# tayloraswift/swift-png

Hardware: AMD Instinct MI355X
Metric: decoded_mpixels_per_s (higher is better)
Workload: dtype u8

## Files before the change

### swift_png_amd/csrc/pinflate2.hip

```cpp
#include "common.hpp"
#include <type_traits>
#include <cstddef>
#include "huffman.hpp"

namespace spng {

#ifdef SPNG_EMU
#define AS_GLOBAL
#else
#define AS_GLOBAL __attribute__((address_space(1)))
#endif
__device__ __forceinline__ uint32_t mul24(uint32_t a, uint32_t b)
{
#ifdef SPNG_EMU
    return (a & 0xffffffu) * (b & 0xffffffu);
#else
    uint32_t r;
    asm("v_mul_u32_u24 %0, %1, %2" : "=v"(r) : "v"(a), "v"(b));
    return r;
#endif
}
typedef uint32_t v4u __attribute__((vector_size(16)));
struct __attribute__((packed)) PV4 { v4u v; };
typedef uint8_t AS_GLOBAL g8;
// ... 1061 lines not shown
__global__ __launch_bounds__(64) void pinf2_cutplan_kernel(PStream *__restrict__ streams, PSeg *__restrict__ segs, PCut *__restrict__ cuts, uint32_t *__restrict__ stats)
{
    __shared__ __attribute__((aligned(16))) DLds s;
    const int lane = threadIdx.x;
    PStream &st = streams[blockIdx.x];
    const uint32_t need = UNI(st.cut_segs);
    if (!need || UNI(st.serial_only)) return;
    const uint32_t first = UNI(st.seg_first), count = UNI(st.seg_count);
    const g8 *src = (const g8 *)uni64((uint64_t)st.src);
    const uint64_t n = uni64(st.src_len), sb = uni64(st.seg_bytes), org = uni64(st.seg_origin);
    const bool rcut = UNI(st.cut_resumed) != 0;
    {
        uint32_t prev = ~0u;
        for (uint32_t base = 0; base < count; base += 64) {
            const uint32_t i = base + (uint32_t)lane;
            unsigned long long mask = __ballot(i < count && segs[first + i].start_bit != NONE2);
            while (mask) {
                const uint32_t f = base + (uint32_t)__ffsll((long long)mask) - 1;
                mask &= mask - 1;
                bool keep = true;
                if (prev != ~0u && f - prev - 1 >= need) {
                    const uint64_t at = uni64(segs[first + f].start_bit);
                    Hdr2 h;
                    if (UB(parse_header2(s, src, n, uni64(segs[first + prev].start_bit), h, lane)) && h.type != 0) {
                        uint32_t len = 0, code = 0;
                        for (uint32_t k = 0; k < (1u << LB) / 64; ++k) {
                            const uint32_t idx = k * 64 + (uint32_t)lane, e = s.lit[idx];
                            const unsigned long long m = __ballot(((e >> 5) & 7) == C_EOB);
                            if (m && !len) {
                                const int l = __ffsll((long long)m) - 1;
                                len = (uint32_t)__shfl((int)((e >> 8) & 15), l, 64);
                                code = (k * 64 + (uint32_t)l) & ((1u << len) - 1);
                            }
                        }
                        if (len && at >= len) {
                            const uint64_t b = at - len;
                            uint32_t v = 0;
                            for (uint32_t k = 0; k < 3; ++k) if ((b >> 3) + k < n) v |= (uint32_t)src[(b >> 3) + k] << (8 * k);
                            keep = ((v >> (b & 7)) & ((1u << len) - 1)) == code;
                        }
                    }
                }
                if (keep) prev = f;
                else if (lane == 0) segs[first + f].start_bit = NONE2;
            }
        }
        __threadfence();
    }
    uint32_t carry = ~0u;
    for (uint32_t base = 0; base < count; base += 64) {
        const uint32_t i = base + (uint32_t)lane;
        const bool has = i < count && segs[first + i].start_bit != NONE2;
        const unsigned long long mask = __ballot(has);
        const unsigned long long low = mask & ((2ull << lane) - 1);
        if (i < count) cuts[first + i].anchor = low ? base + 63 - (uint32_t)__clzll((long long)low) : carry;
        if (mask) carry = base + 63 - (uint32_t)__clzll((long long)mask);
    }
    uint32_t nxt = count, tried = 0;
    for (uint32_t base = (count - 1) & ~63u;; base -= 64) {
        const uint32_t i = base + (uint32_t)lane;
        const bool has = i < count && segs[first + i].start_bit != NONE2;
        const unsigned long long mask = __ballot(has);
        const unsigned long long high = mask >> lane;
        const uint32_t nf = high ? i + (uint32_t)__ffsll((long long)high) - 1 : nxt;
        bool cut = false;
        if (i < count && !has) {
            const uint32_t a = cuts[first + i].anchor;
            if (a != ~0u) {
                const uint64_t lo = org + (uint64_t)(a + 1) * sb, hi = org + (uint64_t)nf * sb < n ? org + (uint64_t)nf * sb : n;
                const uint64_t b = segs[first + a].start_bit;
                const uint64_t from = a == 0 && rcut ? org : lo;
                if (hi > lo && hi - from >= (uint64_t)need * sb && b + 3 <= n * 8) {
                    const uint32_t v = (uint32_t)src[b >> 3] | ((b >> 3) + 1 < n ? (uint32_t)src[(b >> 3) + 1] << 8 : 0u);
                    const uint32_t type = (v >> ((b & 7) + 1)) & 3;
                    cut = type == 1 || type == 2;
                }
            }
            cuts[first + i].cut = cut ? 1u : 0u;
        }
        tried += (uint32_t)__popcll(__ballot(cut));
        if (mask) nxt = base + (uint32_t)__ffsll((long long)mask) - 1;
        if (base == 0) break;
    }
    if (lane == 0 && tried) { atomicAdd(stats, tried); st.cut_on = 1; }
    if (!tried && uni64(st.tok_bit)) back_to_the_header(st, segs, lane);
}

__global__ __launch_bounds__(64, SPNG_D_WAVES) void pinf2_cutjoin_kernel(const PStream *__restrict__ streams, PSeg *__restrict__ segs,
                                                                        PCut *__restrict__ cuts, uint32_t *__restrict__ pt_slab, DPool pool, uint32_t seg0,
                                                                        uint32_t *__restrict__ stats)
{
    __shared__ __attribute__((aligned(16))) DLds s;
    const int lane = threadIdx.x;
    const PSeg &pd = segs[seg0 + blockIdx.x];
    PCut &pc = cuts[seg0 + blockIdx.x];
    if ((int32_t)UNI(pd.status) != PSEG_CUT) return;
    const PStream &st = streams[UNI(pd.stream)];
    const uint32_t j = UNI(pd.next);
    if (j <= UNI(pd.index) || j >= UNI(st.seg_count)) return;
    const PCut &sg = cuts[UNI(st.seg_first) + j];
    const uint32_t nrec = UNI(sg.nrec);
    if (!UNI(sg.cut) || !nrec) return;
    const g8 *src = (const g8 *)uni64((uint64_t)st.src);
    const uint64_t n = uni64(st.src_len);
    const uint64_t want = uni64(sg.head_tbl);
    uint64_t pos = uni64(pd.end_bit), id = uni64(pc.tbl_id);
    g32 *pt = (g32 *)(pt_slab + uni64(pd.log_off));
    const uint32_t pt_cap = uni64(pd.log_cap) > 0xffffff00ull ? 0xffffff00u : (uint32_t)uni64(pd.log_cap);
    Cursor cur;
    cur.nhw = uni64(pd.ntok); cur.npages = (uint32_t)((cur.nhw + PAGE_HW - 1) >> (PAGE_SHIFT - 1)); cur.dry = false;
    cur.pa = (cur.nhw & (PAGE_HW - 1)) ? (g8 *)(pool.base + ((uint64_t)UNI(pt[cur.nhw >> (PAGE_SHIFT - 1)]) << PAGE_SHIFT)) : nullptr;
    const uint64_t hw0 = cur.nhw;
    uint64_t nbytes = 0;
    uint32_t c = 0, chunks = 0;
    bool mid = true, have = false, ok = false;
    uint64_t jt = 0, jt_bytes = 0;
    Hdr2 h;
    for (uint32_t steps = 0; steps < 4 * CUT_JOIN_CHUNKS; ++steps) {
        while (c < nrec && uni64(sg.rec[c].bit) < pos) ++c;
        if (c == nrec) break;
        if (mid && uni64(sg.rec[c].bit) == pos) { ok = id == want; break; }
        if (chunks == CUT_JOIN_CHUNKS) break;
        if (!have || !mid) {
            const uint64_t at = mid ? uni64(pc.tbl) : pos;
            if (!UB(parse_header2(s, src, n, at, h, lane)) || h.type == 0) break;
            have = true;
            if (!mid) { id = table_id(h, pos); jt = pos; jt_bytes = nbytes; pos = h.payload; mid = true; continue; }
        }
        const uint32_t sdw = chunk_dwords(h.minlen);
        const uint64_t chb = (uint64_t)sdw * 32 * 64, upto = uni64(sg.rec[c].bit);
        uint64_t next;
        const uint32_t state = cut_chunk<true>(s, h, src, n, pos, pos, sdw, pool, pt, pt_cap, cur, next, nbytes, upto - pos < chb ? upto : pos + chb, lane);
        chunks += 1;
        if (state == 2) break;
        pos = uni64(next);
        if (state == 1) { if (h.bfinal) break; mid = false; }
    }
    if (!ok) return;
    if (chunks > 1) COV(7);
    if (lane == 0) {
        pc.add_tok = cur.nhw - hw0; pc.add_bytes = nbytes;
        pc.next_head = UNI(sg.rec[c].hw); pc.next_sub = UNI(sg.rec[c].bytes); pc.joined = 1;
        pc.next_bit = pos; pc.join_tbl = jt; pc.join_tbl_bytes = jt_bytes;
        atomicAdd(stats + 1, 1u);
    }
}

template <uint32_t RETRY, bool CUT>
__device__ __forceinline__ void scan_stream(PStream *__restrict__ streams, PSeg *__restrict__ segs, PPart *__restrict__ parts, uint32_t *__restrict__ stats,
                                            const PCut *__restrict__ cuts)
{
    constexpr uint32_t retry = RETRY;
    const int lane = threadIdx.x;
    PStream &st = streams[blockIdx.x];
    if (retry && UNI(st.pass) != 1) {
        if (lane == 0) st.ok = 0;
        return;
    }
    const uint32_t first = UNI(st.seg_first), count = UNI(st.seg_count);
    bool ok = false, partial = false, dry = false;
    uint64_t tok = 0, end_bit = 0, out = 0;
    uint32_t k = 0;
    bool met_cut = false, by_cut = false;
    uint32_t skip_hw = 0; uint64_t skip_bytes = 0;
    const bool rcut = CUT && UNI(st.cut_resumed) != 0;
    uint64_t cur_hdr = CUT ? uni64(st.start_bit) : 0, cur_out = CUT ? uni64(st.blk_out) : 0, ho_bit = 0;
    bool handed = false;
    for (uint32_t hops = 0; hops < count; ++hops) {
        PSeg *sg = segs + first + k;
        const uint64_t start = uni64(sg->start_bit), end = uni64(sg->end_bit);
        const int32_t status = (int32_t)UNI(sg->status);
        if (status == PSEG_NOPAGE && (start != NONE2 || (CUT && by_cut))) dry = true;
        if ((start == NONE2 && !(CUT && by_cut)) || status == PSEG_FAIL || status == PSEG_NOPAGE) break;
        if constexpr (CUT) {
            uint64_t nt = uni64(sg->ntok), nb = uni64(sg->nbytes);
            const uint32_t hd = by_cut ? skip_hw : 0u;
            if (by_cut) nb -= skip_bytes;
            uint32_t nx = 0;
            if (status == PSEG_CUT) {
                met_cut = true;
                nx = UNI(sg->next);
                const PCut &ct = cuts[first + k];
                const bool joined = nx > k && nx < count && UNI(cuts[first + nx].cut) && UNI(ct.joined);
                if (rcut) {
                    if (UNI(ct.tbl_here)) { cur_hdr = uni64(ct.tbl); cur_out = uni64(st.out_pos) + out + uni64(ct.tbl_bytes) - (by_cut ? skip_bytes : 0); }
                    if (!joined || (int32_t)UNI(segs[first + nx].status) == PSEG_FAIL) {
                        ho_bit = end;
                        if (joined) {
                            if (uni64(ct.join_tbl)) { cur_hdr = uni64(ct.join_tbl); cur_out = uni64(st.out_pos) + out + nb + uni64(ct.join_tbl_bytes); }
                            nt += uni64(ct.add_tok); nb += uni64(ct.add_bytes); ho_bit = uni64(ct.next_bit);
                        }
                        if (lane == 0) { sg->tok_base = tok; sg->out_base = out; sg->used = 1; sg->ntok = nt; sg->nbytes = nb; sg->head = hd; sg->status = PSEG_PARTIAL; }
                        tok += nt - hd; out += nb;
                        handed = true;
                        break;
                    }
                    if (uni64(ct.join_tbl)) { cur_hdr = uni64(ct.join_tbl); cur_out = uni64(st.out_pos) + out + nb + uni64(ct.join_tbl_bytes); }
                }
                if (!joined) break;
                nt += uni64(ct.add_tok); nb += uni64(ct.add_bytes);
                skip_hw = UNI(ct.next_head); skip_bytes = uni64(ct.next_sub);
            }
            if (lane == 0) { sg->tok_base = tok; sg->out_base = out; sg->used = 1; sg->ntok = nt; sg->nbytes = nb; sg->head = hd; }
            tok += nt - hd;
            out += nb;
            if (status == PSEG_CUT) { k = nx; by_cut = true; continue; }
            by_cut = false;
        } else {
        if (lane == 0) { sg->tok_base = tok; sg->out_base = out; sg->used = 1; }
        tok += uni64(sg->ntok);
        out += uni64(sg->nbytes);
        }
        if (status == PSEG_FINAL) { ok = true; end_bit = end; break; }
        if (status == PSEG_PARTIAL) { ok = true; partial = true; end_bit = end; break; }
        const uint32_t nx = UNI(sg->next);
        if (nx <= k || nx >= count) break;
        if (uni64(segs[first + nx].start_bit) != end) break;
        k = nx;
    }
    if (CUT && handed && uni64(st.src_len) * 8 - ho_bit <= 2 * uni64(st.seg_bytes) * 8) { ok = true; partial = true; end_bit = ho_bit; }
    else handed = false;
    if (CUT && met_cut && !(ok && (!partial || rcut))) {
        ok = false; partial = false; dry = true; handed = false;
        if (lane == 0) atomicAdd(stats + 2, 1u);
        COV(8);
    }
    bool again = !retry && dry;
    if constexpr (CUT) { if (again && uni64(st.tok_bit)) again = back_to_the_header(st, segs, lane); }
    const uint32_t pmax = UNI(st.parts_max);
    uint32_t np = 0;
    if (pmax > 1 && ok && uni64(st.start_bit) == 0 && uni64(st.out_pos) == 0 && out <= uni64(st.dst_cap) && out > 0) {
        PPart *pp = parts + (uint64_t)blockIdx.x * pmax;
        uint64_t w0 = (uint64_t)gridDim.x * (pmax - 1) > 256 ? 1 : 0;
#ifdef SPNG_EMU
        if (getenv("EMU_FIRST_PART_SHARE")) w0 = 1;
#endif
        uint64_t begun = 0;
        uint32_t kk = 0, tnext = 1;
        np = 1;
        if (lane == 0) { pp[0].seg = 0; pp[0].out_pos = 0; pp[0].present = 1; }
        for (uint32_t hops = 0; hops < count; ++hops) {
            const PSeg *sg = segs + first + kk;
            const uint64_t ob = uni64(sg->out_base);
            if (kk != 0 && tnext < pmax && ob >= 32768u && ob > begun && ob * (2 * pmax + w0) >= (uint64_t)(2 * tnext + w0) * out) {
                if (lane == 0) {
                    pp[np].seg = kk; pp[np].out_pos = ob; pp[np].present = 1;
                    pp[np - 1].seg_end = kk; pp[np - 1].out_len = ob - begun;
                }
                begun = ob; np += 1;
                tnext = (uint32_t)((ob * (2 * pmax + w0) / out + 2 - w0) / 2);
            }
            if ((int32_t)UNI(sg->status) == PSEG_FINAL || (int32_t)UNI(sg->status) == PSEG_PARTIAL) break;
            kk = UNI(sg->next);
        }
        if (lane == 0) { pp[np - 1].seg_end = ~0u; pp[np - 1].out_len = out - begun; }
    }
    if (lane == 0) { st.ok = ok ? (handed ? 3 : partial ? 2 : 1) : 0; st.ntok = tok; st.end_bit = end_bit; st.pass = again ? 1 : 0; st.tok_base = 0;
                     st.out_total = out; st.parts = np; st.ho_hdr = cur_hdr; st.ho_out = cur_out; }
}

template <uint32_t RETRY>
__global__ __launch_bounds__(64) void pinf2_scan_kernel(PStream *__restrict__ streams, PSeg *__restrict__ segs, PPart *__restrict__ parts)
{
    scan_stream<RETRY, false>(streams, segs, parts, nullptr, nullptr);
}
__global__ __launch_bounds__(64) void pinf2_cutscan_kernel(PStream *__restrict__ streams, PSeg *__restrict__ segs, const PCut *__restrict__ cuts,
                                                           PPart *__restrict__ parts, uint32_t *__restrict__ stats)
{
    scan_stream<0, true>(streams, segs, parts, stats, cuts);
}

#ifndef SPNG_R_THREADS
#define SPNG_R_THREADS 512
#define SPNG_R_WAVES 4
#endif
static constexpr uint32_t RT2 = SPNG_R_THREADS;
static constexpr uint32_t NW2 = RT2 / 64;
template <bool BIG> struct RGeo {
    static constexpr uint32_t TILE = BIG ? 8192 : 4096;
    static constexpr uint32_t BPT = TILE / RT2;
    static constexpr uint32_t HPT = TILE / 2 / RT2;
    static constexpr uint32_t EB = BPT < 8 ? BPT : 8;
    static constexpr uint32_t MAXM = TILE / 8;
};
static constexpr uint32_t WINDOW2 = 32768;
static constexpr uint32_t R2_DONE = 0x8000;
static constexpr uint32_t PTC = 256;

template <bool MARK> struct RingOf { typedef uint8_t T; };
template <> struct RingOf<true> { typedef uint16_t T; };
template <bool MARK, bool BIG>
struct RLds2T {
    typename RingOf<MARK>::T ring[WINDOW2];
    uint16_t state[RGeo<BIG>::TILE];
    uint32_t rec[RGeo<BIG>::MAXM + 2][2];
    uint32_t bitmap[RGeo<BIG>::TILE / 32];
    uint16_t h0[RT2 + 8];
    uint32_t pt[PTC];
    uint32_t part[3 * NW2];
    uint32_t cut[2];
};

template <class L>
__device__ __forceinline__ uint32_t block_excl_scan2(L &s, uint32_t v, uint32_t &total, int tid)
{
    const int lane = tid & 63, wave = tid >> 6;
    uint32_t wt;
    const uint32_t off = wave_excl_scan(v, wt, lane);
    if (lane == 0) s.part[wave] = wt;
    __syncthreads();
    uint32_t before = 0, all = 0;
#pragma unroll
    for (int w4 = 0; w4 < (int)NW2; w4 += 4) {
        const v4u p = *(const v4u *)(s.part + w4);
#pragma unroll
        for (int c = 0; c < 4; ++c) { before += w4 + c < wave ? p[c] : 0u; all += p[c]; }
    }
    total = all;
    return off + before;
}

__device__ __forceinline__ void stream_verdict(const PStream &st, uint32_t S, uint32_t I, uint64_t pos, spng_result *__restrict__ results,
                                               int32_t *__restrict__ done)
{
    const g8 *src = (const g8 *)st.src;
    const uint64_t n = st.src_len;
    uint64_t *state = st.state;
    const bool whole = st.start_bit == 0 && st.out_pos == 0;
    if (st.ok == 2 || st.ok == 3) {
        const bool tok = st.ok == 3;
        state[0] = tok ? st.ho_hdr : st.end_bit; state[1] = tok ? st.ho_out : pos; state[2] = tok ? st.end_bit : 0; state[3] = tok ? pos : 0;
    } else if (!whole) {
        const uint64_t endb = (st.end_bit + 7) / 8, consumed = endb + (st.format == SPNG_FORMAT_ZLIB ? 4 : 0);
        spng_result &res = results[st.image];
        if (consumed <= n) {
            res.status = SPNG_DONE; res.reserved = 1;
            res.written = pos; res.consumed = consumed;
            res.aux[0] = res.aux[1] = 0;
            *done = 1;
        }
    } else {
        const uint64_t endb = (st.end_bit + 7) / 8;
        spng_result &res = results[st.image];
        if (st.format == SPNG_FORMAT_IOS) {
            res.status = SPNG_DONE; res.reserved = 1;
            res.written = pos; res.consumed = endb;
            res.aux[0] = res.aux[1] = 0;
            *done = 1;
        } else if (endb + 4 <= n) {
            const uint32_t declared = (uint32_t)src[endb] << 24 | (uint32_t)src[endb + 1] << 16 |
                                      (uint32_t)src[endb + 2] << 8 | (uint32_t)src[endb + 3];
            const uint32_t N = (uint32_t)(pos % 65521);
            const uint32_t computed = (uint32_t)((N + (uint64_t)N * S % 65521 + 65521 - I) % 65521) << 16 | (1 + S) % 65521;
            res.status = declared == computed ? SPNG_DONE : SPNG_E_STREAM_CHECKSUM; res.reserved = 1;
            res.written = pos; res.consumed = endb + 4;
            res.aux[0] = declared == computed ? 0 : declared; res.aux[1] = declared == computed ? 0 : computed;
            *done = 1;
        }
    }
}

template <uint32_t RETRY, bool MARK, bool BIG>
__global__ __launch_bounds__(RT2, SPNG_R_WAVES) void pinf2_resolve_kernel(const PStream *__restrict__ streams, const PSeg *__restrict__ segs,
                                                               const uint32_t *__restrict__ pt_slab, DPool pool,
                                                               spng_result *__restrict__ results, int32_t *__restrict__ done,
                                                               PPart *__restrict__ parts, uint32_t pmax, uint16_t *__restrict__ sym)
{
    constexpr uint32_t retry = RETRY;
    constexpr uint32_t TILE2 = RGeo<BIG>::TILE, BPT2 = RGeo<BIG>::BPT, HPT2 = RGeo<BIG>::HPT, EB2 = RGeo<BIG>::EB, MAXM2 = RGeo<BIG>::MAXM;
    static_assert(HPT2 == 8 || HPT2 == 4, "a thread's halfwords of a window are one 16- or 8-byte load");
    constexpr uint32_t DONE = MARK ? 0x4000u : R2_DONE;
    constexpr uint32_t KNOWN = MARK ? 0xc000u : R2_DONE;
    __shared__ __attribute__((aligned(16))) RLds2T<MARK, BIG> s;
    const int tid = threadIdx.x, lane = tid & 63, wave = (int)UNI((uint32_t)tid >> 6);
    const uint32_t sidx = MARK ? blockIdx.x / (pmax - 1) : blockIdx.x;
    const uint32_t pidx = MARK ? 1 + blockIdx.x % (pmax - 1) : 0;
    const PStream &st = streams[sidx];
    if (!UNI(st.ok) || (retry && done[sidx])) return;
    const uint32_t nparts = pmax ? UNI(st.parts) : 0;
    if (MARK && pidx >= nparts) return;
    PPart *part = nparts > 1 ? parts + (uint64_t)sidx * pmax + pidx : nullptr;
    const uint32_t seg_end = part ? UNI(part->seg_end) : ~0u;
    const uint64_t part_pos = part ? uni64(part->out_pos) : 0;
    g8 *dst = (g8 *)uni64((uint64_t)st.dst);
    const uint64_t cap = uni64(st.dst_cap);
    uint64_t pos = uni64(st.out_pos) + part_pos;
    uint32_t accS = 0, accI = 0;
    uint32_t pmod = (uint32_t)(pos % 65521);
    bool bad = false, over = false;
    g16 *symo = MARK ? (g16 *)(sym + uni64(st.sym_off)) : nullptr;
    if (!MARK && pos) {
        for (uint64_t p = (pos > WINDOW2 ? pos - WINDOW2 : 0) + (uint32_t)tid; p < pos; p += RT2) s.ring[p & (WINDOW2 - 1)] = dst[p];
    }
    if (tid < (int)(TILE2 / 32)) s.bitmap[tid] = 0;
    if (tid == 0) { s.rec[0][0] = 0; s.rec[0][1] = 1; }
    __syncthreads();
    const uint32_t seg_first = UNI(st.seg_first), seg_count = UNI(st.seg_count);
    uint32_t sk = part ? UNI(part->seg) : 0;
#ifdef SPNG_D_PROF
    uint64_t rp[12] = {0, 0, 0, 0, 0, 0, 0, 0, 0, 0, 0, 0}, rp_t = __builtin_readcyclecounter();
#define RP2(k) do { const uint64_t now_ = __builtin_readcyclecounter(); rp[k] += now_ - rp_t; rp_t = now_; } while (0)
#define RPN2(k, v) (rp[k] += (v))
#else
#define RP2(k)
#define RPN2(k, v)
#endif
    constexpr uint32_t NULL2 = TK_NULL | TK_NULL << 16;
    for (uint32_t hops = 0; hops < seg_count && !over && sk != seg_end; ++hops) {
        const PSeg &sg = segs[seg_first + sk];
        const uint64_t nhw = uni64(sg.ntok);
        const g32 *ptg = (const g32 *)(pt_slab + uni64(sg.log_off));
        const int32_t sstatus = (int32_t)UNI(sg.status);
        uint64_t cursor = UNI(sg.head);
        uint64_t pt_lo = 0;
        __syncthreads();
        for (uint32_t i = (uint32_t)tid; i < PTC; i += RT2) s.pt[i] = (pt_lo + i) * PAGE_UNITS * 8 < nhw + 8 ? ptg[pt_lo + i] : 0u;
        __syncthreads();
        uint32_t tv[HPT2 / 2];
        auto load_window = [&](uint64_t from) {
            const uint64_t h = (from & ~(uint64_t)(HPT2 - 1)) + (uint64_t)tid * HPT2;
#pragma unroll
            for (int k = 0; k < (int)(HPT2 / 2); ++k) tv[k] = NULL2;
            if (h < nhw) {
                const uint64_t u = h >> 3;
                const uint32_t pid = s.pt[(u >> (PAGE_SHIFT - 4)) - pt_lo];
                const g8 *q = (const g8 *)pool.base + ((uint64_t)pid << PAGE_SHIFT) + ((u & (PAGE_UNITS - 1)) << 4) + ((h & 7) << 1);
                if constexpr (HPT2 == 8) { const v4u v = ((const gPV4 *)q)->v; tv[0] = v[0]; tv[1] = v[1]; tv[2] = v[2]; tv[3] = v[3]; }
                else { const v2u v = ((const gPV2 *)q)->v; tv[0] = v[0]; tv[1] = v[1]; }
            }
        };
        load_window(cursor);
        while (cursor < nhw) {
            RP2(0);
            const uint64_t wb = cursor;
            uint32_t hh[HPT2];
#pragma unroll
            for (int j = 0; j < (int)HPT2; ++j) {
                const uint32_t idx = (uint32_t)tid * HPT2 + j;
                const uint32_t v = (tv[j >> 1] >> (16 * (j & 1))) & 0xffff;
                hh[j] = wb + idx < nhw ? v : TK_NULL;
            }
            s.h0[tid] = (uint16_t)hh[0];
            if (tid == 0) s.cut[1] = 0xffffffffu;
            uint32_t bytes = 0, refs = 0;
#pragma unroll
            for (int j = 0; j < (int)HPT2; ++j) {
                const uint32_t v = hh[j];
                const bool lit = !(v & 0x8000), m0 = (v & 0xC000) == 0x8000;
                bytes += lit ? 1u : m0 ? (v & 0xff) + 3 : 0u;
                refs += m0 ? 1u : 0u;
            }
            uint32_t total;
            const uint32_t offp = block_excl_scan2(s, refs << 20 | bytes, total, tid);
            RP2(1);
            uint32_t curb = offp & 0xfffff, curm = offp >> 20;
            const uint32_t hnext = tid + 1 < (int)RT2 ? s.h0[tid + 1] : TK_NULL;
            const bool front = curb <= TILE2 && curm <= MAXM2;
            const bool fits = curb + bytes <= TILE2 && curm + refs <= MAXM2 &&
                              !(tid == (int)RT2 - 1 && (hh[HPT2 - 1] & 0xC000) == 0x8000);
            if (front && !fits) { s.cut[0] = curb; s.cut[1] = (uint32_t)tid * HPT2; if (curb + bytes <= TILE2 && curm + refs > MAXM2) COV(9); }
            if (fits) {
#pragma unroll
                for (int j = 0; j < (int)HPT2; ++j) {
                    const uint32_t v = hh[j];
                    if (!(v & 0x8000)) { s.state[curb] = (uint16_t)(DONE | v); curb += 1; }
                    else if ((v & 0xC000) == 0x8000) {
                        const uint32_t len = (v & 0xff) + 3;
                        const uint32_t h1 = j < (int)HPT2 - 1 ? hh[j < (int)HPT2 - 1 ? j + 1 : (int)HPT2 - 1] : hnext;
                        const uint32_t dd = (((v >> 8) & 63) | (h1 & 0x1ff) << 6) + 1;
                        atomicOr(&s.bitmap[curb >> 5], 1u << (curb & 31));
                        s.rec[curm + 1][0] = curb | len << 16;
                        s.rec[curm + 1][1] = dd;
                        curb += len; curm += 1;
                    }
                }
            }
            __syncthreads();
            const uint32_t cut0 = s.cut[0], cut1 = s.cut[1];
            const uint64_t wend = nhw - wb < (uint64_t)RT2 * HPT2 ? nhw - wb : (uint64_t)RT2 * HPT2;
            const uint32_t tlen = cut1 != 0xffffffffu ? cut0 : total & 0xfffff;
            const uint32_t wlast = cut1 != 0xffffffffu ? cut1 : (uint32_t)wend;
            if (pos + tlen > cap) { over = true; break; }
            const uint64_t cursor_next = wb + wlast;
            if ((((cursor_next + 2 * RT2 * HPT2) >> 3) >> (PAGE_SHIFT - 4)) >= pt_lo + PTC) {
                __syncthreads();
                pt_lo = (cursor_next >> 3) >> (PAGE_SHIFT - 4);
                for (uint32_t i = (uint32_t)tid; i < PTC; i += RT2) s.pt[i] = (pt_lo + i) * PAGE_UNITS * 8 < nhw + 8 ? ptg[pt_lo + i] : 0u;
                __syncthreads();
            }
            load_window(cursor_next);
            RP2(2);
            const uint32_t rbase = (uint32_t)pos & (WINDOW2 - 1);
            const bool early = pos - part_pos < WINDOW2;
            uint32_t sv[BPT2];
            {
                v4u bw = {0, 0, 0, 0};
                if ((uint32_t)lane < TILE2 / 128) bw = *(const v4u *)(s.bitmap + 4 * lane);
                const uint32_t ca = (uint32_t)__popc(bw[0]) + (uint32_t)__popc(bw[1]), cbb = (uint32_t)__popc(bw[2]) + (uint32_t)__popc(bw[3]);
                uint32_t tt;
                const uint32_t rb = wave_excl_scan(ca + cbb, tt, lane);
                const bool odd = wave & 1;
                const uint32_t srclo = odd ? bw[2] : bw[0], srchi = odd ? bw[3] : bw[1], srcbase = odd ? rb + ca : rb;
                auto expand_rows = [&](auto early_c) {
                constexpr bool EARLY = decltype(early_c)::value;
#pragma unroll
                for (int part = 0; part < (int)(BPT2 / EB2); ++part) {
                    v2u recv[EB2];
#pragma unroll
                    for (int kk = 0; kk < (int)EB2; ++kk) {
                        const int k = part * (int)EB2 + kk;
                        const uint32_t row = (uint32_t)wave + NW2 * k;
                        const uint32_t mlo = (uint32_t)__builtin_amdgcn_readlane((int)srclo, (int)(row >> 1));
                        const uint32_t mhi = (uint32_t)__builtin_amdgcn_readlane((int)srchi, (int)(row >> 1));
                        const uint32_t base = (uint32_t)__builtin_amdgcn_readlane((int)srcbase, (int)(row >> 1));
                        const unsigned long long mw1 = ((unsigned long long)mhi << 32 | mlo) >> 1;
                        const uint32_t id = __builtin_amdgcn_mbcnt_hi((uint32_t)(mw1 >> 32), __builtin_amdgcn_mbcnt_lo((uint32_t)mw1, base + (mlo & 1)));
                        recv[kk] = *(const v2u *)s.rec[id];
                    }
                    uint32_t siv[EB2], farv[EB2];
#pragma unroll
                    for (int kk = 0; kk < (int)EB2; ++kk) {
                        const int k = part * (int)EB2 + kk;
                        const uint32_t j = ((uint32_t)wave + NW2 * k) * 64 + (uint32_t)lane;
                        const uint32_t startb = recv[kk][0] & 0xffff, len = recv[kk][0] >> 16, d = recv[kk][1];
                        uint32_t kk2 = j - startb;
                        const bool inside = kk2 < len;
                        if (inside && kk2 >= d) COV(10);
                        if (inside && kk2 >= d) kk2 -= mul24(d, (uint32_t)(((float)kk2 + 0.5f) * __builtin_amdgcn_rcpf((float)d)));
                        if (inside && kk2 >= d) COV(12);
                        siv[kk] = inside ? startb - d + kk2 : 0x7fffffffu;
                        farv[kk] = s.ring[(rbase + siv[kk]) & (WINDOW2 - 1)];
                    }
#pragma unroll
                    for (int kk = 0; kk < (int)EB2; ++kk) {
                        const int k = part * (int)EB2 + kk;
                        const uint32_t j = ((uint32_t)wave + NW2 * k) * 64 + (uint32_t)lane;
                        const uint32_t si = siv[kk];
                        sv[k] = DONE;
                        if (si != 0x7fffffffu) {
                            uint32_t v;
                            if (MARK) {
                                const uint32_t rel = (uint32_t)(pos - part_pos) + si;
                                v = (int32_t)si >= 0 ? si : (!EARLY || (int32_t)rel >= 0) ? farv[kk] : 0x8000u | (rel + WINDOW2);
                                if (EARLY && (int32_t)si < 0 && (int32_t)rel < 0) COV(11);
                            } else {
                                if (EARLY && (int32_t)si < 0 && (uint32_t)pos < 0u - si) bad = true;
                                v = (int32_t)si < 0 ? DONE | farv[kk] : si;
                            }
                            sv[k] = v;
                            s.state[j] = (uint16_t)v;
                        }
                    }
                }
                };
                if (early) expand_rows(std::true_type{}); else expand_rows(std::false_type{});
            }
            __syncthreads();
            RP2(3);
            if (tid < (int)(TILE2 / 32)) s.bitmap[tid] = 0;
            for (;;) {
                asm volatile("" ::: "memory");
                bool more = false;
                uint32_t gv[BPT2];
#pragma unroll
                for (int k = 0; k < (int)BPT2; ++k) { gv[k] = DONE; if (!(sv[k] & KNOWN)) gv[k] = s.state[sv[k]]; }
#pragma unroll
                for (int k = 0; k < (int)BPT2; ++k) {
                    if (!(sv[k] & KNOWN)) {
                        const uint32_t j = ((uint32_t)wave + NW2 * k) * 64 + (uint32_t)lane;
                        sv[k] = gv[k]; s.state[j] = (uint16_t)gv[k]; more = more || !(gv[k] & KNOWN);
                    }
                }
                RPN2(9, 1);
                if (!__ballot(more)) break;
            }
            __syncthreads();
            RP2(4);
            {
                uint32_t bv[BPT2];
#pragma unroll
                for (int k = 0; k < (int)BPT2; ++k) bv[k] = s.state[((uint32_t)wave + NW2 * k) * 64 + (uint32_t)lane];
#pragma unroll
                for (int k = 0; k < (int)BPT2; ++k) {
                    const uint32_t j = ((uint32_t)wave + NW2 * k) * 64 + (uint32_t)lane;
                    if (j < tlen) s.ring[(rbase + j) & (WINDOW2 - 1)] = (typename RingOf<MARK>::T)bv[k];
                }
            }
            __syncthreads();
            if constexpr (MARK) {
                const uint64_t u0 = pos >> 3, u1 = (pos + tlen) >> 3;
                for (uint64_t u = u0 + (uint32_t)tid; u < u1; u += RT2) {
                    const uint16_t *r = s.ring + ((u << 3) & (WINDOW2 - 1));
                    if ((u << 3) >= part_pos) ((gPV4 *)(symo + (u << 3)))->v = *(const v4u *)r;
                    else for (int c = 0; c < 8; ++c) if ((u << 3) + c >= part_pos) symo[(u << 3) + c] = r[c];
                }
            } else {
                const uint64_t u0 = pos >> 4, u1 = (pos + tlen) >> 4;
                for (uint64_t u = u0 + (uint32_t)tid; u < u1; u += RT2) {
                    const v4u v = *(const v4u *)(s.ring + ((u << 4) & (WINDOW2 - 1)));
                    ((gPV4 *)(dst + (u << 4)))->v = v;
                    uint32_t A = 0, J = 0;
                    A = __builtin_amdgcn_sad_u8(v[0], 0, A); A = __builtin_amdgcn_sad_u8(v[1], 0, A);
                    A = __builtin_amdgcn_sad_u8(v[2], 0, A); A = __builtin_amdgcn_sad_u8(v[3], 0, A);
                    J = __builtin_amdgcn_udot4(v[0], 0x03020100u, J, false);
                    J = __builtin_amdgcn_udot4(v[1], 0x07060504u, J, false);
                    J = __builtin_amdgcn_udot4(v[2], 0x0b0a0908u, J, false);
                    J = __builtin_amdgcn_udot4(v[3], 0x0f0e0d0cu, J, false);
                    const uint32_t g = (pmod + 65521u - ((uint32_t)pos & 15u) + 16u * (uint32_t)(u - u0)) % 65521u;
                    accS = (accS + A) % 65521u;
                    accI = (accI + g * A + J) % 65521u;
                }
            }
            pos += tlen;
            pmod = (pmod + tlen) % 65521u;
            cursor = cursor_next;
            RP2(5);
            RPN2(8, 1); RPN2(10, tlen);
        }
        if (sstatus == PSEG_FINAL || sstatus == PSEG_PARTIAL) break;
        sk = UNI(sg.next);
    }
#ifdef SPNG_D_PROF
    if (blockIdx.x == 0 && (tid == 0 || tid == 300))
        printf("resolve[t%d]: %lu tiles (%lu bytes), %lu rounds; cycles: loop %lu window+scan %lu take+prefetch %lu expand %lu jump %lu store %lu\n",
               tid, rp[8], rp[10], rp[9], rp[0], rp[1], rp[2], rp[3], rp[4], rp[5]);
#endif
    __syncthreads();
    if constexpr (MARK) {
        const uint64_t u1 = pos >> 3 << 3, at = u1 + (uint32_t)tid;
        if (!over && at < pos && at >= part_pos) symo[at] = s.ring[at & (WINDOW2 - 1)];
    } else {
        const uint64_t u1 = pos >> 4 << 4;
        if (!over && u1 + (uint32_t)tid < pos) {
            const uint32_t b = s.ring[(u1 + (uint32_t)tid) & (WINDOW2 - 1)];
            dst[u1 + (uint32_t)tid] = (uint8_t)b;
            const uint32_t g = (uint32_t)((u1 + (uint32_t)tid) % 65521);
            accS = (accS + b) % 65521;
            accI = (uint32_t)((accI + (uint64_t)g * b) % 65521);
        }
    }
    if (__syncthreads_or(bad || over)) {
        if (part && tid == 0) part->failed = 1;
        return;
    }
    if constexpr (MARK) return;
    else {
        const uint32_t S1 = wave_sum(accS) % 65521, I1 = wave_sum(accI % 65521) % 65521;
        __syncthreads();
        if (lane == 0) { s.part[wave] = S1; s.part[NW2 + wave] = I1; }
        __syncthreads();
        uint32_t S = 0, I = 0;
        for (int w = 0; w < (int)NW2; ++w) { S += s.part[w]; I += s.part[NW2 + w]; }
        S %= 65521; I %= 65521;
        if (part) {
            if (tid == 0) { part->sumS = S; part->sumI = I; }
            return;
        }
        if (tid == 0) stream_verdict(st, S, I, pos, results, done + sidx);
    }
}

__global__ __launch_bounds__(512) void pinf2_window_kernel(const PStream *__restrict__ streams, const PPart *__restrict__ parts, uint32_t pmax,
                                                           const uint16_t *__restrict__ sym, uint8_t *__restrict__ win)
{
    const PStream &st = streams[blockIdx.x];
    const uint32_t np = UNI(st.parts);
    if (!UNI(st.ok) || np < 2) return;
    const PPart *pp = parts + (uint64_t)blockIdx.x * pmax;
    const g8 *dst = (const g8 *)uni64((uint64_t)st.dst);
    const g16 *symo = (const g16 *)(sym + uni64(st.sym_off));
    g8 *w = (g8 *)win + (uint64_t)blockIdx.x * pmax * WINDOW2;
    for (uint32_t p = 1; p < np; ++p) {
        const uint64_t from = uni64(pp[p].out_pos) - WINDOW2, before = uni64(pp[p - 1].out_pos);
        for (uint32_t o = threadIdx.x; o < WINDOW2; o += 512) {
            const uint64_t a = from + o;
            uint32_t b;
            if (p == 1) b = dst[a];
            else if (a >= before) {
                const uint32_t v = symo[a];
                b = v & 0x8000 ? w[(uint64_t)(p - 1) * WINDOW2 + (v & 0x7fff)] : v & 0xff;
            } else b = w[(uint64_t)(p - 1) * WINDOW2 + (uint32_t)(a - (before - WINDOW2))];
            w[(uint64_t)p * WINDOW2 + o] = (uint8_t)b;
        }
        __threadfence();
        __syncthreads();
    }
}

static constexpr uint32_t FIX_WG = 32;
__global__ __launch_bounds__(256) void pinf2_fixup_kernel(const PStream *__restrict__ streams, PPart *__restrict__ parts, uint32_t pmax,
                                                          const uint16_t *__restrict__ sym, const uint8_t *__restrict__ win)
{
    const uint32_t sidx = blockIdx.y / (pmax - 1), pidx = 1 + blockIdx.y % (pmax - 1);
    const PStream &st = streams[sidx];
    if (!UNI(st.ok) || pidx >= UNI(st.parts)) return;
    PPart &part = parts[(uint64_t)sidx * pmax + pidx];
    if (UNI(part.failed)) return;
    const uint64_t p0 = uni64(part.out_pos), p1 = p0 + uni64(part.out_len);
    g8 *dst = (g8 *)uni64((uint64_t)st.dst);
    const g16 *symo = (const g16 *)(sym + uni64(st.sym_off));
    const g8 *w = (const g8 *)win + ((uint64_t)sidx * pmax + pidx) * WINDOW2;
    unsigned long long S = 0, I = 0;
    const uint64_t u0 = p0 >> 3, u1 = (p1 + 7) >> 3;
    for (uint64_t u = u0 + (uint64_t)blockIdx.x * 256 + threadIdx.x; u < u1; u += (uint64_t)FIX_WG * 256) {
        const uint64_t at = u << 3;
        const bool inner = at >= p0 && at + 8 <= p1;
        uint32_t b[8];
        if (inner) {
            const v4u v = ((const gPV4 *)(symo + at))->v;
#pragma unroll
            for (int c = 0; c < 8; ++c) b[c] = (v[c >> 1] >> (16 * (c & 1))) & 0xffff;
        } else {
#pragma unroll
            for (int c = 0; c < 8; ++c) b[c] = (at + c >= p0 && at + c < p1) ? (uint32_t)symo[at + c] : 0x4000u;
        }
#pragma unroll
        for (int c = 0; c < 8; ++c) b[c] = b[c] & 0x8000 ? (uint32_t)w[b[c] & 0x7fff] : b[c] & 0xff;
        if (inner) {
            v2u o;
            o[0] = b[0] | b[1] << 8 | b[2] << 16 | b[3] << 24; o[1] = b[4] | b[5] << 8 | b[6] << 16 | b[7] << 24;
            ((gPV2 *)(dst + at))->v = o;
        } else {
#pragma unroll
            for (int c = 0; c < 8; ++c) if (at + c >= p0 && at + c < p1) dst[at + c] = (uint8_t)b[c];
        }
        const uint32_t g = (uint32_t)(at % 65521);
#pragma unroll
        for (int c = 0; c < 8; ++c) {
            const bool mine = inner || (at + c >= p0 && at + c < p1);
            const uint32_t v = mine ? b[c] : 0u;
            S += v; I += (unsigned long long)((g + (uint32_t)c) % 65521u) * v;
        }
    }
#pragma unroll
    for (int m = 32; m >= 1; m >>= 1) {
        S += (unsigned long long)(uint32_t)__shfl_xor((int)(uint32_t)S, m, 64) | (unsigned long long)(uint32_t)__shfl_xor((int)(uint32_t)(S >> 32), m, 64) << 32;
        I += (unsigned long long)(uint32_t)__shfl_xor((int)(uint32_t)I, m, 64) | (unsigned long long)(uint32_t)__shfl_xor((int)(uint32_t)(I >> 32), m, 64) << 32;
    }
    if ((threadIdx.x & 63) == 0) { atomicAdd(&part.sumS, S); atomicAdd(&part.sumI, I); }
}

__global__ void pinf2_verdict_kernel(const PStream *__restrict__ streams, const PPart *__restrict__ parts, uint32_t pmax,
                                     spng_result *__restrict__ results, int32_t *__restrict__ done, uint32_t count)
{
    const uint32_t i = blockIdx.x * blockDim.x + threadIdx.x;
    if (i >= count) return;
    const PStream &st = streams[i];
    if (!st.ok || st.parts < 2 || done[i]) return;
    const PPart *pp = parts + (uint64_t)i * pmax;
    unsigned long long S = 0, I = 0;
    for (uint32_t p = 0; p < st.parts; ++p) {
        if (pp[p].failed) return;
        S = (S + pp[p].sumS % 65521) % 65521; I = (I + pp[p].sumI % 65521) % 65521;
    }
    stream_verdict(st, (uint32_t)S, (uint32_t)I, st.out_total, results, done + i);
}

__global__ void pinf2_account_kernel(uint32_t *ctr, uint32_t *totals, uint32_t pages)
{
    const uint32_t used = ctr[0];
    atomicAdd(&totals[0], used < pages ? used : pages);
    if (used >= pages) atomicOr(&totals[1], 1u);
    atomicAdd(&totals[2], ctr[1]); ctr[1] = 0;
}

#ifndef SPNG_EMU
hipError_t launch_pinf2_find(PStream *d_streams, PSeg *d_segs, uint32_t seg0, uint32_t nsegs, uint32_t retry, hipStream_t stream)
{
    if (retry) pinf2_find_kernel<1><<<nsegs, 64, 0, stream>>>(d_streams, d_segs, seg0);
    else pinf2_find_kernel<0><<<nsegs, 64, 0, stream>>>(d_streams, d_segs, seg0);
    return hipGetLastError();
}
hipError_t launch_pinf2_decode(PStream *d_streams, PSeg *d_segs, uint32_t seg0, uint32_t nsegs, uint32_t *d_pt, uint8_t *d_pool, uint32_t *d_next,
                               uint32_t pages, uint32_t retry, hipStream_t stream)
{
    DPool pool{d_pool, d_next, pages, 0};
    if (retry) pinf2_decode_kernel<1><<<nsegs, 64, 0, stream>>>(d_streams, d_segs, d_pt, pool, seg0);
    else pinf2_decode_kernel<0><<<nsegs, 64, 0, stream>>>(d_streams, d_segs, d_pt, pool, seg0);
    return hipGetLastError();
}
hipError_t launch_pinf2_cutplan(PStream *d_streams, uint32_t nstreams, PSeg *d_segs, PCut *d_cuts, uint32_t *d_stats, hipStream_t stream)
{
    pinf2_cutplan_kernel<<<nstreams, 64, 0, stream>>>(d_streams, d_segs, d_cuts, d_stats);
    return hipGetLastError();
}
hipError_t launch_pinf2_cutdecode(PStream *d_streams, PSeg *d_segs, PCut *d_cuts, uint32_t seg0, uint32_t nsegs, uint32_t *d_pt, uint8_t *d_pool,
                                  uint32_t *d_next, uint32_t pages, hipStream_t stream)
{
    DPool pool{d_pool, d_next, pages, 0};
    pinf2_cutdecode_kernel<1><<<nsegs, 64, 0, stream>>>(d_streams, d_segs, d_pt, pool, seg0, d_cuts);
    pinf2_cutdecode_kernel<2><<<nsegs, 64, 0, stream>>>(d_streams, d_segs, d_pt, pool, seg0, d_cuts);
    return hipGetLastError();
}
hipError_t launch_pinf2_cutjoin(PStream *d_streams, PSeg *d_segs, PCut *d_cuts, uint32_t seg0, uint32_t nsegs, uint32_t *d_pt, uint8_t *d_pool,
                                uint32_t *d_next, uint32_t pages, uint32_t *d_stats, hipStream_t stream)
{
    DPool pool{d_pool, d_next, pages, 0};
    pinf2_cutjoin_kernel<<<nsegs, 64, 0, stream>>>(d_streams, d_segs, d_cuts, d_pt, pool, seg0, d_stats);
    return hipGetLastError();
}
hipError_t launch_pinf2_cutscan(PStream *d_streams, uint32_t nstreams, PSeg *d_segs, PCut *d_cuts, PPart *d_parts, uint32_t *d_stats, hipStream_t stream)
{
    pinf2_cutscan_kernel<<<nstreams, 64, 0, stream>>>(d_streams, d_segs, d_cuts, d_parts, d_stats);
    return hipGetLastError();
}
hipError_t launch_pinf2_scan(PStream *d_streams, uint32_t nstreams, PSeg *d_segs, PPart *d_parts, uint32_t retry, hipStream_t stream)
{
    if (retry) pinf2_scan_kernel<1><<<nstreams, 64, 0, stream>>>(d_streams, d_segs, d_parts);
    else pinf2_scan_kernel<0><<<nstreams, 64, 0, stream>>>(d_streams, d_segs, d_parts);
    return hipGetLastError();
}
hipError_t launch_pinf2_resolve(PStream *d_streams, uint32_t nstreams, PSeg *d_segs, uint32_t *d_pt, uint8_t *d_pool, uint32_t pages,
                                spng_result *d_results, int32_t *d_done, PPart *d_parts, uint32_t pmax, uint32_t retry, hipStream_t stream)
{
    DPool pool{d_pool, nullptr, pages, 0};
    if (retry) pinf2_resolve_kernel<1, false, true><<<nstreams, RT2, 0, stream>>>(d_streams, d_segs, d_pt, pool, d_results, d_done, d_parts, pmax, nullptr);
    else pinf2_resolve_kernel<0, false, true><<<nstreams, RT2, 0, stream>>>(d_streams, d_segs, d_pt, pool, d_results, d_done, d_parts, pmax, nullptr);
    return hipGetLastError();
}
hipError_t launch_pinf2_parts(PStream *d_streams, uint32_t nstreams, PSeg *d_segs, uint32_t *d_pt, uint8_t *d_pool, uint32_t pages,
                              spng_result *d_results, int32_t *d_done, PPart *d_parts, uint32_t pmax, uint16_t *d_sym, hipStream_t stream)
{
    DPool pool{d_pool, nullptr, pages, 0};
    if (nstreams * (pmax - 1) > 256) pinf2_resolve_kernel<0, true, false><<<nstreams * (pmax - 1), RT2, 0, stream>>>(d_streams, d_segs, d_pt, pool, d_results, d_done, d_parts, pmax, d_sym);
    else pinf2_resolve_kernel<0, true, true><<<nstreams * (pmax - 1), RT2, 0, stream>>>(d_streams, d_segs, d_pt, pool, d_results, d_done, d_parts, pmax, d_sym);
    return hipGetLastError();
}
hipError_t launch_pinf2_join(PStream *d_streams, uint32_t nstreams, spng_result *d_results, int32_t *d_done, PPart *d_parts, uint32_t pmax,
                             uint16_t *d_sym, uint8_t *d_win, hipStream_t stream)
{
    pinf2_window_kernel<<<nstreams, 512, 0, stream>>>(d_streams, d_parts, pmax, d_sym, d_win);
    pinf2_fixup_kernel<<<dim3(FIX_WG, nstreams * (pmax - 1)), 256, 0, stream>>>(d_streams, d_parts, pmax, d_sym, d_win);
    pinf2_verdict_kernel<<<(nstreams + 63) / 64, 64, 0, stream>>>(d_streams, d_parts, pmax, d_results, d_done, nstreams);
    return hipGetLastError();
}
hipError_t launch_pinf2_account(uint32_t *d_ctr, uint32_t *d_totals, uint32_t pages, hipStream_t stream)
{
    pinf2_account_kernel<<<1, 1, 0, stream>>>(d_ctr, d_totals, pages);
    return hipGetLastError();
}
#endif

}
```

Before: 35580.

## Defer tile output store and pipeline next window's scan to cut barriers

Splits the block scan into contribute and collect phases so the next window's token classification and wave scan run before the end-of-tile barrier. The global store and Adler accumulation of a finished tile are deferred into the next iteration, where they overlap with token placement. Two __syncthreads per tile are removed. In exchange it adds UPT vector registers per thread and relies on the ring contents staying valid until the deferred read. Profiling labels are updated to match.

```diff
diff --git a/swift_png_amd/csrc/pinflate2.hip b/swift_png_amd/csrc/pinflate2.hip
--- a/swift_png_amd/csrc/pinflate2.hip
+++ b/swift_png_amd/csrc/pinflate2.hip
@@ -1387,13 +1387,18 @@
 };
 
 template <class L>
-__device__ __forceinline__ uint32_t block_excl_scan2(L &s, uint32_t v, uint32_t &total, int tid)
+__device__ __forceinline__ uint32_t block_scan2_contribute(L &s, uint32_t v, int tid)
 {
     const int lane = tid & 63, wave = tid >> 6;
     uint32_t wt;
     const uint32_t off = wave_excl_scan(v, wt, lane);
     if (lane == 0) s.part[wave] = wt;
-    __syncthreads();
+    return off;
+}
+template <class L>
+__device__ __forceinline__ uint32_t block_scan2_collect(const L &s, uint32_t off, uint32_t &total, int tid)
+{
+    const int wave = tid >> 6;
     uint32_t before = 0, all = 0;
 #pragma unroll
     for (int w4 = 0; w4 < (int)NW2; w4 += 4) {
@@ -1491,6 +1496,46 @@
 #define RPN2(k, v)
 #endif
     constexpr uint32_t NULL2 = TK_NULL | TK_NULL << 16;
+    constexpr uint32_t UB = MARK ? 8 : 16;
+    constexpr uint32_t UPT = TILE2 / UB / RT2;
+    static_assert(UPT * UB * RT2 == TILE2 && UPT >= 1, "a tile's units are UPT per thread");
+    uint64_t d_pos = 0;
+    uint32_t d_len = 0, d_pmod = 0;
+    v4u dv[UPT];
+    auto deferred_read = [&]() {
+        const uint64_t u0 = d_pos / UB, u1 = (d_pos + d_len) / UB;
+#pragma unroll
+        for (int i = 0; i < (int)UPT; ++i) {
+            const uint64_t u = u0 + (uint32_t)tid + (uint32_t)i * RT2;
+            if (u < u1) dv[i] = *(const v4u *)(s.ring + ((u * UB) & (WINDOW2 - 1)));
+        }
+    };
+    auto deferred_write = [&]() {
+        const uint64_t u0 = d_pos / UB, u1 = (d_pos + d_len) / UB;
+#pragma unroll
+        for (int i = 0; i < (int)UPT; ++i) {
+            const uint64_t u = u0 + (uint32_t)tid + (uint32_t)i * RT2;
+            if (u >= u1) continue;
+            const v4u v = dv[i];
+            if constexpr (MARK) {
+                if ((u << 3) >= part_pos) ((gPV4 *)(symo + (u << 3)))->v = v;
+                else for (int c = 0; c < 8; ++c) if ((u << 3) + c >= part_pos) symo[(u << 3) + c] = (uint16_t)(v[c >> 1] >> (16 * (c & 1)));
+            } else {
+                ((gPV4 *)(dst + (u << 4)))->v = v;
+                uint32_t A = 0, J = 0;
+                A = __builtin_amdgcn_sad_u8(v[0], 0, A); A = __builtin_amdgcn_sad_u8(v[1], 0, A);
+                A = __builtin_amdgcn_sad_u8(v[2], 0, A); A = __builtin_amdgcn_sad_u8(v[3], 0, A);
+                J = __builtin_amdgcn_udot4(v[0], 0x03020100u, J, false);
+                J = __builtin_amdgcn_udot4(v[1], 0x07060504u, J, false);
+                J = __builtin_amdgcn_udot4(v[2], 0x0b0a0908u, J, false);
+                J = __builtin_amdgcn_udot4(v[3], 0x0f0e0d0cu, J, false);
+                const uint32_t g = (d_pmod + 65521u - ((uint32_t)d_pos & 15u) + 16u * (uint32_t)(u - u0)) % 65521u;
+                accS = (accS + A) % 65521u;
+                accI = (accI + g * A + J) % 65521u;
+            }
+        }
+        d_len = 0;
+    };
     for (uint32_t hops = 0; hops < seg_count && !over && sk != seg_end; ++hops) {
         const PSeg &sg = segs[seg_first + sk];
         const uint64_t nhw = uni64(sg.ntok);
@@ -1514,11 +1559,8 @@
                 else { const v2u v = ((const gPV2 *)q)->v; tv[0] = v[0]; tv[1] = v[1]; }
             }
         };
-        load_window(cursor);
-        while (cursor < nhw) {
-            RP2(0);
-            const uint64_t wb = cursor;
-            uint32_t hh[HPT2];
+        uint32_t hh[HPT2], bytes = 0, refs = 0, woff = 0;
+        auto contribute = [&](uint64_t wb) {
 #pragma unroll
             for (int j = 0; j < (int)HPT2; ++j) {
                 const uint32_t idx = (uint32_t)tid * HPT2 + j;
@@ -1527,7 +1569,7 @@
             }
             s.h0[tid] = (uint16_t)hh[0];
             if (tid == 0) s.cut[1] = 0xffffffffu;
-            uint32_t bytes = 0, refs = 0;
+            bytes = 0; refs = 0;
 #pragma unroll
             for (int j = 0; j < (int)HPT2; ++j) {
                 const uint32_t v = hh[j];
@@ -1535,9 +1577,17 @@
                 bytes += lit ? 1u : m0 ? (v & 0xff) + 3 : 0u;
                 refs += m0 ? 1u : 0u;
             }
+            woff = block_scan2_contribute(s, refs << 20 | bytes, tid);
+        };
+        load_window(cursor);
+        if (cursor < nhw) { contribute(cursor); __syncthreads(); }
+        while (cursor < nhw) {
+            RP2(0);
+            const uint64_t wb = cursor;
             uint32_t total;
-            const uint32_t offp = block_excl_scan2(s, refs << 20 | bytes, total, tid);
+            const uint32_t offp = block_scan2_collect(s, woff, total, tid);
             RP2(1);
+            deferred_read();
             uint32_t curb = offp & 0xfffff, curm = offp >> 20;
             const uint32_t hnext = tid + 1 < (int)RT2 ? s.h0[tid + 1] : TK_NULL;
             const bool front = curb <= TILE2 && curm <= MAXM2;
@@ -1560,7 +1610,10 @@
                     }
                 }
             }
+            deferred_write();
+            RP2(2);
             __syncthreads();
+            RP2(6);
             const uint32_t cut0 = s.cut[0], cut1 = s.cut[1];
             const uint64_t wend = nhw - wb < (uint64_t)RT2 * HPT2 ? nhw - wb : (uint64_t)RT2 * HPT2;
             const uint32_t tlen = cut1 != 0xffffffffu ? cut0 : total & 0xfffff;
@@ -1574,7 +1627,6 @@
                 __syncthreads();
             }
             load_window(cursor_next);
-            RP2(2);
             const uint32_t rbase = (uint32_t)pos & (WINDOW2 - 1);
             const bool early = pos - part_pos < WINDOW2;
             uint32_t sv[BPT2];
@@ -1640,8 +1692,9 @@
                 };
                 if (early) expand_rows(std::true_type{}); else expand_rows(std::false_type{});
             }
+            RP2(3);
             __syncthreads();
-            RP2(3);
+            RP2(6);
             if (tid < (int)(TILE2 / 32)) s.bitmap[tid] = 0;
             for (;;) {
                 asm volatile("" ::: "memory");
@@ -1659,8 +1712,6 @@
                 RPN2(9, 1);
                 if (!__ballot(more)) break;
             }
-            __syncthreads();
-            RP2(4);
             {
                 uint32_t bv[BPT2];
 #pragma unroll
@@ -1671,31 +1722,11 @@
                     if (j < tlen) s.ring[(rbase + j) & (WINDOW2 - 1)] = (typename RingOf<MARK>::T)bv[k];
                 }
             }
+            if (cursor_next < nhw) contribute(cursor_next);
+            RP2(4);
             __syncthreads();
-            if constexpr (MARK) {
-                const uint64_t u0 = pos >> 3, u1 = (pos + tlen) >> 3;
-                for (uint64_t u = u0 + (uint32_t)tid; u < u1; u += RT2) {
-                    const uint16_t *r = s.ring + ((u << 3) & (WINDOW2 - 1));
-                    if ((u << 3) >= part_pos) ((gPV4 *)(symo + (u << 3)))->v = *(const v4u *)r;
-                    else for (int c = 0; c < 8; ++c) if ((u << 3) + c >= part_pos) symo[(u << 3) + c] = r[c];
-                }
-            } else {
-                const uint64_t u0 = pos >> 4, u1 = (pos + tlen) >> 4;
-                for (uint64_t u = u0 + (uint32_t)tid; u < u1; u += RT2) {
-                    const v4u v = *(const v4u *)(s.ring + ((u << 4) & (WINDOW2 - 1)));
-                    ((gPV4 *)(dst + (u << 4)))->v = v;
-                    uint32_t A = 0, J = 0;
-                    A = __builtin_amdgcn_sad_u8(v[0], 0, A); A = __builtin_amdgcn_sad_u8(v[1], 0, A);
-                    A = __builtin_amdgcn_sad_u8(v[2], 0, A); A = __builtin_amdgcn_sad_u8(v[3], 0, A);
-                    J = __builtin_amdgcn_udot4(v[0], 0x03020100u, J, false);
-                    J = __builtin_amdgcn_udot4(v[1], 0x07060504u, J, false);
-                    J = __builtin_amdgcn_udot4(v[2], 0x0b0a0908u, J, false);
-                    J = __builtin_amdgcn_udot4(v[3], 0x0f0e0d0cu, J, false);
-                    const uint32_t g = (pmod + 65521u - ((uint32_t)pos & 15u) + 16u * (uint32_t)(u - u0)) % 65521u;
-                    accS = (accS + A) % 65521u;
-                    accI = (accI + g * A + J) % 65521u;
-                }
-            }
+            RP2(6);
+            d_pos = pos; d_len = tlen; d_pmod = pmod;
             pos += tlen;
             pmod = (pmod + tlen) % 65521u;
             cursor = cursor_next;
@@ -1707,9 +1738,11 @@
     }
 #ifdef SPNG_D_PROF
     if (blockIdx.x == 0 && (tid == 0 || tid == 300))
-        printf("resolve[t%d]: %lu tiles (%lu bytes), %lu rounds; cycles: loop %lu window+scan %lu take+prefetch %lu expand %lu jump %lu store %lu\n",
-               tid, rp[8], rp[10], rp[9], rp[0], rp[1], rp[2], rp[3], rp[4], rp[5]);
+        printf("resolve[t%d]: %lu tiles (%lu bytes), %lu rounds; cycles: loop %lu collect %lu take+store %lu prefetch+expand %lu jump+copy+scan %lu barrier waits %lu\n",
+               tid, rp[8], rp[10], rp[9], rp[0] + rp[5], rp[1], rp[2], rp[3], rp[4], rp[6]);
 #endif
+    deferred_read();
+    deferred_write();
     __syncthreads();
     if constexpr (MARK) {
         const uint64_t u1 = pos >> 3 << 3, at = u1 + (uint32_t)tid;
```

Result: no change. 35810, median of 6 (+0.6%).
